# jeremy-rifkin/Markov-Huffman-Coding

Hardware: AMD Instinct MI355X
Metric: encode+decode GB/s on 16 GB byte stream, bit-exact round-trip (higher is better)
Workload: dtype u8

## Files before the change

### markov-huffman-coding_amd/csrc/mh_tree.hip

```cpp
#include <hip/hip_runtime.h>
#include <stdint.h>

#include "mh_kernels.h"
#include "mh_model.hpp"

namespace mhk {

using mh::DEC16_LEAF;
using mh::DEC16_NULL;
using mh::TREE_LEAF;
using mh::TREE_STRIDE;

constexpr uint16_t NONE = 0xFFFF;

template <bool K64>
struct RegHeap {
    uint32_t klo[10], khi[10], itm[10];
    uint32_t hn = 0;

    static __device__ __forceinline__ uint32_t uni(uint32_t v) { return uint32_t(__builtin_amdgcn_readfirstlane(int(v))); }
    static __device__ __forceinline__ uint32_t rl(uint32_t v, uint32_t lane) { return uint32_t(__builtin_amdgcn_readlane(int(v), int(lane))); }
    static __device__ __forceinline__ uint32_t wl(uint32_t val, uint32_t lane, uint32_t old) {
#pragma clang diagnostic push
#pragma clang diagnostic ignored "-Winline-asm"
        asm("s_mov_b32 m0, %2\n\tv_writelane_b32 %0, %1, m0" : "+v"(old) : "s"(uni(val)), "s"(uni(lane)) : "m0");
#pragma clang diagnostic pop
        return old;
    }
    static __device__ __forceinline__ bool lt(uint32_t alo, uint32_t ahi, uint32_t blo, uint32_t bhi) {
        if (K64) return ahi < bhi || (ahi == bhi && alo < blo);
        return alo < blo;
    }
    template <int L>
    __device__ __forceinline__ void get(uint32_t pos, uint32_t &lo, uint32_t &hi, uint32_t &it) const {
        if constexpr (L < 7) {
            lo = rl(klo[L], pos); hi = K64 ? rl(khi[L], pos) : 0u; it = rl(itm[L], pos);
        } else if constexpr (L == 7) {
            const uint32_t ln = pos & 63u;
            const bool up = pos >= 64u;
            lo = up ? rl(klo[8], ln) : rl(klo[7], ln);
            hi = K64 ? (up ? rl(khi[8], ln) : rl(khi[7], ln)) : 0u;
            it = up ? rl(itm[8], ln) : rl(itm[7], ln);
        } else {
            lo = rl(klo[9], 0); hi = K64 ? rl(khi[9], 0) : 0u; it = rl(itm[9], 0);
        }
    }
    template <int L>
    __device__ __forceinline__ void put(uint32_t pos, uint32_t lo, uint32_t hi, uint32_t it) {
        if constexpr (L < 7) {
            klo[L] = wl(lo, pos, klo[L]); if (K64) khi[L] = wl(hi, pos, khi[L]); itm[L] = wl(it, pos, itm[L]);
        } else if constexpr (L == 7) {
            const uint32_t ln = pos & 63u;
            if (pos >= 64u) { klo[8] = wl(lo, ln, klo[8]); if (K64) khi[8] = wl(hi, ln, khi[8]); itm[8] = wl(it, ln, itm[8]); }
            else { klo[7] = wl(lo, ln, klo[7]); if (K64) khi[7] = wl(hi, ln, khi[7]); itm[7] = wl(it, ln, itm[7]); }
        } else {
            klo[9] = wl(lo, 0, klo[9]); if (K64) khi[9] = wl(hi, 0, khi[9]); itm[9] = wl(it, 0, itm[9]);
        }
    }

    template <int L>
    __device__ __forceinline__ void swim_flat(uint32_t pos, uint32_t lo, uint32_t hi, uint32_t it) {
        uint32_t alo[L + 1], ahi[L + 1], ait[L + 1];
        uint32_t moves = 0;
        bool going = true;
        alo[L] = lo; ahi[L] = hi; ait[L] = it;
#pragma unroll
        for (int l = L - 1; l >= 0; --l) {
            get_dyn(l, pos >> (L - l), alo[l], ahi[l], ait[l]);
            going = going && lt(lo, hi, alo[l], ahi[l]);
            moves += going ? 1u : 0u;
        }
        const uint32_t f = uint32_t(L) - moves;
#pragma unroll
        for (int l = L; l >= 0; --l) {
            const bool from_parent = uint32_t(l) > f;
            const bool self = uint32_t(l) < f;
            const uint32_t plo = l > 0 ? alo[l > 0 ? l - 1 : 0] : lo, phi = l > 0 ? ahi[l > 0 ? l - 1 : 0] : hi,
                           pit = l > 0 ? ait[l > 0 ? l - 1 : 0] : it;
            const uint32_t wlo = from_parent ? plo : self ? alo[l] : lo;
            const uint32_t whi = from_parent ? phi : self ? ahi[l] : hi;
            const uint32_t wit = from_parent ? pit : self ? ait[l] : it;
            put_dyn(l, pos >> (L - l), wlo, whi, wit);
        }
    }
    template <int L>
    __device__ __forceinline__ void swim_short(uint32_t pos, uint32_t lo, uint32_t hi, uint32_t it) {
        uint32_t alo[L + 1], ahi[L + 1], ait[L + 1];
        uint32_t moves = 0;
#pragma unroll
        for (int l = L - 1; l >= 0; --l) {
            get_dyn(l, pos >> (L - l), alo[l], ahi[l], ait[l]);
            if (!lt(lo, hi, alo[l], ahi[l])) break;
            ++moves;
        }
#pragma unroll
        for (int m = 0; m < L; ++m) {
            if (uint32_t(m) < moves) put_dyn(L - m, pos >> m, alo[L - 1 - m], ahi[L - 1 - m], ait[L - 1 - m]);
        }
        put_any_level<L>(L - moves, pos >> moves, lo, hi, it);
    }
    template <int L>
    __device__ __forceinline__ void put_any_level(uint32_t level, uint32_t pos, uint32_t lo, uint32_t hi, uint32_t it) {
        switch (level) {
            case 0: put<0>(pos, lo, hi, it); break;
            case 1: if (L >= 1) put<1>(pos, lo, hi, it); break;
            case 2: if (L >= 2) put<2>(pos, lo, hi, it); break;
            case 3: if (L >= 3) put<3>(pos, lo, hi, it); break;
            case 4: if (L >= 4) put<4>(pos, lo, hi, it); break;
            case 5: if (L >= 5) put<5>(pos, lo, hi, it); break;
            case 6: if (L >= 6) put<6>(pos, lo, hi, it); break;
            case 7: if (L >= 7) put<7>(pos, lo, hi, it); break;
            default: if (L >= 8) put<8>(pos, lo, hi, it); break;
        }
    }
    __device__ __forceinline__ void get_dyn(int l, uint32_t pos, uint32_t &lo, uint32_t &hi, uint32_t &it) const {
        switch (l) {
            case 0: get<0>(pos, lo, hi, it); break; case 1: get<1>(pos, lo, hi, it); break; case 2: get<2>(pos, lo, hi, it); break;
            case 3: get<3>(pos, lo, hi, it); break; case 4: get<4>(pos, lo, hi, it); break; case 5: get<5>(pos, lo, hi, it); break;
            case 6: get<6>(pos, lo, hi, it); break; case 7: get<7>(pos, lo, hi, it); break; default: get<8>(pos, lo, hi, it); break;
        }
    }
    __device__ __forceinline__ void put_dyn(int l, uint32_t pos, uint32_t lo, uint32_t hi, uint32_t it) {
        switch (l) {
            case 0: put<0>(pos, lo, hi, it); break; case 1: put<1>(pos, lo, hi, it); break; case 2: put<2>(pos, lo, hi, it); break;
            case 3: put<3>(pos, lo, hi, it); break; case 4: put<4>(pos, lo, hi, it); break; case 5: put<5>(pos, lo, hi, it); break;
            case 6: put<6>(pos, lo, hi, it); break; case 7: put<7>(pos, lo, hi, it); break; default: put<8>(pos, lo, hi, it); break;
        }
    }
    __device__ __forceinline__ void push(uint32_t lo, uint32_t hi, uint32_t it) {
        const uint32_t i = hn++;
        const uint32_t level = 31u - uint32_t(__builtin_clz(i + 1u));
        const uint32_t pos = i + 1u - (1u << level);
        switch (level) {
            case 0: swim_short<0>(pos, lo, hi, it); break;
            case 1: swim_short<1>(pos, lo, hi, it); break;
            case 2: swim_short<2>(pos, lo, hi, it); break;
            case 3: swim_short<3>(pos, lo, hi, it); break;
            case 4: swim_short<4>(pos, lo, hi, it); break;
            case 5: swim_short<5>(pos, lo, hi, it); break;
            case 6: swim_short<6>(pos, lo, hi, it); break;
            case 7: swim_short<7>(pos, lo, hi, it); break;
            default: swim_short<8>(pos, lo, hi, it); break;
        }
    }
    template <int LMAX>
    __device__ __forceinline__ void sink_flat(uint32_t lo, uint32_t hi, uint32_t it) {
        uint32_t pos[LMAX + 1], clo[LMAX + 1], chi[LMAX + 1], cit[LMAX + 1];
        pos[0] = 0; clo[0] = lo; chi[0] = hi; cit[0] = it;
        uint32_t moves = 0;
        bool going = true;
#pragma unroll
        for (int l = 0; l < LMAX; ++l) {
            const uint32_t li = ((2u << l) - 1u) + 2u * pos[l];
            uint32_t llo, lhi, lit, rlo, rhi, rit;
            get_dyn(l + 1, 2u * pos[l], llo, lhi, lit);
            get_dyn(l + 1, 2u * pos[l] + 1u, rlo, rhi, rit);
            const bool right = li + 1u < hn && lt(rlo, rhi, llo, lhi);
            clo[l + 1] = right ? rlo : llo; chi[l + 1] = right ? rhi : lhi; cit[l + 1] = right ? rit : lit;
            pos[l + 1] = 2u * pos[l] + (right ? 1u : 0u);
            going = going && li < hn && lt(clo[l + 1], chi[l + 1], lo, hi);
            moves += going ? 1u : 0u;
        }
#pragma unroll
        for (int l = 0; l <= LMAX; ++l) {
            const bool from_child = uint32_t(l) < moves;
            const bool self = uint32_t(l) > moves;
            const int c = l < LMAX ? l + 1 : LMAX;
            const uint32_t wlo = from_child ? clo[c] : self ? clo[l] : lo;
            const uint32_t whi = from_child ? chi[c] : self ? chi[l] : hi;
            const uint32_t wit = from_child ? cit[c] : self ? cit[l] : it;
            put_dyn(l, pos[l], wlo, whi, wit);
        }
    }
    __device__ __forceinline__ uint32_t pop(uint32_t &mlo, uint32_t &mhi) {
        uint32_t top;
        get<0>(0, mlo, mhi, top);
        --hn;
        const uint32_t level = 31u - uint32_t(__builtin_clz(hn + 1u));
        const uint32_t pos = hn + 1u - (1u << level);
        uint32_t lo, hi, it;
        switch (level) {
            case 0: get<0>(pos, lo, hi, it); sink_flat<0>(lo, hi, it); break;
            case 1: get<1>(pos, lo, hi, it); sink_flat<1>(lo, hi, it); break;
            case 2: get<2>(pos, lo, hi, it); sink_flat<2>(lo, hi, it); break;
            case 3: get<3>(pos, lo, hi, it); sink_flat<3>(lo, hi, it); break;
            case 4: get<4>(pos, lo, hi, it); sink_flat<4>(lo, hi, it); break;
            case 5: get<5>(pos, lo, hi, it); sink_flat<5>(lo, hi, it); break;
            case 6: get<6>(pos, lo, hi, it); sink_flat<6>(lo, hi, it); break;
            case 7: get<7>(pos, lo, hi, it); sink_flat<7>(lo, hi, it); break;
            default: get<8>(pos, lo, hi, it); sink_flat<8>(lo, hi, it); break;
        }
        return top;
    }
};

struct TreeLds {
    uint16_t *left, *right, *parent, *height;
    uint8_t *sym;
    unsigned long long *weight;
};

template <bool K64>
__device__ __forceinline__ void merge_context(const TreeLds &t, uint32_t nleaf, uint32_t lane, uint32_t &nn_out, uint32_t &root_out,
                                              uint32_t &single_out) {
    RegHeap<K64> h;
#pragma unroll
    for (int i = 0; i < 10; ++i) { h.klo[i] = 0; h.khi[i] = 0; h.itm[i] = 0; }
    for (uint32_t i = 0; i < nleaf; ++i) {
        const unsigned long long w = t.weight[i];
        h.push(RegHeap<K64>::uni(uint32_t(w)), RegHeap<K64>::uni(uint32_t(w >> 32)), i);
    }
    uint32_t nn = nleaf;
    while (h.hn > 1) {
        uint32_t alo, ahi, blo, bhi;
        uint32_t a = h.pop(alo, ahi), b = h.pop(blo, bhi);
        if ((a >> 16) > (b >> 16)) {
            uint32_t x = a; a = b; b = x;
        }
        const unsigned long long w = ((unsigned long long)(ahi) << 32 | alo) + ((unsigned long long)(bhi) << 32 | blo);
        const uint32_t ha = a >> 16, hb = b >> 16, hnew = (ha > hb ? ha : hb) + 1u;
        const uint32_t ia = a & 0xFFFFu, ib = b & 0xFFFFu;
        if (lane == 0) {
            t.left[nn] = uint16_t(ia); t.right[nn] = uint16_t(ib); t.parent[nn] = NONE; t.sym[nn] = 0;
            t.weight[nn] = w; t.height[nn] = uint16_t(hnew);
            t.parent[ia] = t.parent[ib] = uint16_t(nn);
        }
        h.push(uint32_t(w), uint32_t(w >> 32), nn | (hnew << 16));
        ++nn;
    }
    uint32_t rlo, rhi;
    const uint32_t root = h.pop(rlo, rhi) & 0xFFFFu;
    single_out = 0;
    if (nleaf == 1) {
        if (lane == 0) {
            const uint8_t s = t.sym[root];
            for (int k = 0; k < 2; ++k) {
                t.left[nn + k] = t.right[nn + k] = NONE; t.parent[nn + k] = uint16_t(root); t.height[nn + k] = 0; t.sym[nn + k] = s;
                t.weight[nn + k] = t.weight[root];
            }
            t.left[root] = uint16_t(nn); t.right[root] = uint16_t(nn + 1);
            t.height[root] = 1;
        }
        nn += 2;
        single_out = 1;
    }
    nn_out = nn;
    root_out = root;
}

__global__ __launch_bounds__(64) void tree_build_kernel(const unsigned long long *__restrict__ counts, TreeBuildOut o) {
    const uint32_t c = blockIdx.x, lane = threadIdx.x;
    __shared__ unsigned long long cnt[256];
    __shared__ uint16_t left[TB_NODE_STRIDE], right[TB_NODE_STRIDE], parent[TB_NODE_STRIDE], height[TB_NODE_STRIDE];
    __shared__ uint8_t sym[TB_NODE_STRIDE];
    __shared__ unsigned long long weight[TB_NODE_STRIDE];
    __shared__ uint8_t olen[256];
    __shared__ unsigned long long ocode[256];
    __shared__ uint32_t prof[9];
    __shared__ uint32_t s_nn, s_root, s_single, s_ntab8, s_maxlen;

    unsigned long long wsum = 0;
    for (uint32_t i = lane; i < 256; i += 64) {
        cnt[i] = counts[size_t(c) * 256 + i];
        wsum += cnt[i];
        olen[i] = 0;
        ocode[i] = 0;
    }
    for (int d = 32; d >= 1; d >>= 1) wsum += __shfl_xor(wsum, d);
    if (lane < 9) prof[lane] = 0;
    if (lane == 0) { s_ntab8 = 0; s_maxlen = 0; s_single = 0; }
    __syncthreads();

    uint32_t nleaf = 0;
    for (uint32_t i = 0; i < 4; ++i) {
        const uint32_t s = i * 64 + lane;
        const bool nz = cnt[s] != 0;
        const unsigned long long m = __ballot(nz);
        const uint32_t pos = nleaf + __popcll(m & ((1ull << lane) - 1ull));
        if (nz) {
            left[pos] = right[pos] = NONE; parent[pos] = NONE; height[pos] = 0; sym[pos] = uint8_t(s); weight[pos] = cnt[s];
        }
        nleaf += __popcll(m);
    }
    __syncthreads();
    {
        const TreeLds t{left, right, parent, height, sym, weight};
        uint32_t nn = 0, root = 0xFFFFFFFFu, single = 0;
        if (nleaf > 0) {
            const bool wide = uint32_t(__builtin_amdgcn_readfirstlane(int(uint32_t(wsum >> 32)))) != 0;
            if (wide) merge_context<true>(t, nleaf, lane, nn, root, single);
            else merge_context<false>(t, nleaf, lane, nn, root, single);
        }
        if (lane == 0) { s_nn = nn; s_root = root; s_single = single; }
    }
    __syncthreads();

    const uint32_t nn = s_nn, root = s_root;
    if (root != 0xFFFFFFFFu) {
        for (uint32_t node = lane; node < nn; node += 64) {
            uint32_t d = 0;
            unsigned long long code = 0;
            uint32_t cur = node;
            while (cur != root) {
                const uint32_t p = parent[cur];
                if (right[p] == cur && d < 64) code |= 1ull << d;
                ++d;
                cur = p;
            }
            if (left[node] == NONE) {
                if (!(s_single && node == left[root])) {
                    olen[sym[node]] = uint8_t(d > 255 ? 255 : d);
                    ocode[sym[node]] = d <= 64 ? code : 0;
                    atomicMax(&s_maxlen, d);
                }
            } else if (d <= 8) {
                const uint32_t h = height[node] < o.hcap ? height[node] : o.hcap;
                atomicAdd(&prof[d], 1u << h);
                if (d == 8) atomicAdd(&s_ntab8, 1u);
            }
        }
    }
    __syncthreads();

    uint32_t lenmask = 0;
    for (uint32_t s = lane; s < 256; s += 64) {
        const uint32_t l = olen[s];
        if (l) lenmask |= 1u << (l < 32u ? l - 1u : 31u);
        const unsigned long long cd = ocode[s];
        o.len8[c * 256 + s] = uint8_t(l);
        o.code64[c * 256 + s] = cd;
        if (o.enc16) {
            const uint32_t slot = mh::enc_slot((s << 8) | c);
            uint16_t e = 0;
            if (l > uint32_t(mh::ENC16_MAX_LEN)) e = mh::ENC16_ESCAPE;
            else if (l > 0) e = uint16_t((l << 12) | uint32_t(cd));
            o.enc16[slot] = e;
            o.len_slot[slot] = uint8_t(l);
        }
    }
    for (uint32_t i = lane; i < TB_NODE_STRIDE; i += 64) {
        const bool live = i < nn;
        o.node_left[c * TB_NODE_STRIDE + i] = live ? left[i] : NONE;
        o.node_right[c * TB_NODE_STRIDE + i] = live ? right[i] : NONE;
        o.node_sym[c * TB_NODE_STRIDE + i] = live ? sym[i] : 0;
        o.node_height[c * TB_NODE_STRIDE + i] = live ? uint8_t(height[i] > 255 ? 255 : height[i]) : 0;
    }
    for (int d = 32; d >= 1; d >>= 1) lenmask |= __shfl_xor(lenmask, d);
    if (lane == 0) {
        uint32_t *m = o.ctx_meta + c * TB_META_STRIDE;
        m[0] = nn; m[1] = root; m[2] = s_maxlen; m[3] = s_ntab8;
        for (int d = 0; d < 9; ++d) m[4 + d] = prof[d];
        m[13] = uint32_t(wsum); m[14] = uint32_t(wsum >> 32);
        m[15] = nleaf < 2 ? 0u : lenmask;
    }
}

__device__ __forceinline__ void tree_pack_body(const TreePackArgs &a, const uint32_t c) {
    const uint32_t tid = threadIdx.x;
    __shared__ uint16_t left[TB_NODE_STRIDE], right[TB_NODE_STRIDE], nid[TB_NODE_STRIDE];
    __shared__ uint8_t sym[TB_NODE_STRIDE], height[TB_NODE_STRIDE];
    __shared__ uint32_t tr[TREE_STRIDE];
    __shared__ uint32_t scan[256];
    const uint32_t *meta = a.ctx_meta + c * TB_META_STRIDE;
    const uint32_t nn = meta[0], root = meta[1];
    for (uint32_t i = tid; i < TB_NODE_STRIDE; i += 256) {
        left[i] = a.node_left[c * TB_NODE_STRIDE + i];
        right[i] = a.node_right[c * TB_NODE_STRIDE + i];
        sym[i] = a.node_sym[c * TB_NODE_STRIDE + i];
        height[i] = a.node_height[c * TB_NODE_STRIDE + i];
    }
    tr[tid] = 0;
    __syncthreads();
    const uint32_t P = a.P, nprim = 1u << P;
    const uint32_t my_base = a.sec_base_in ? a.sec_base_in[c] : a.sec_base_val[c];
    if (tid == 0 && !a.sec_base_in && a.sec_base) a.sec_base[c] = my_base;
    if (root == 0xFFFFFFFFu) {
        if (tid < nprim) a.prim[(c << P) | tid] = DEC16_NULL;
        if (a.tree) a.tree[c * TREE_STRIDE + tid] = 0;
        return;
    }
    if (tid == 0) {
        uint32_t next = 1;
        for (uint32_t i = 0; i < nn; ++i) nid[i] = (left[i] == NONE) ? NONE : (i == root ? 0 : uint16_t(next++));
    }
    __syncthreads();
    auto enc_child = [&](uint32_t ch) -> uint32_t { return left[ch] == NONE ? (TREE_LEAF | sym[ch]) : uint32_t(nid[ch]); };
    for (uint32_t i = tid; i < nn; i += 256)
        if (left[i] != NONE) tr[nid[i]] = (enc_child(right[i]) << 16) | enc_child(left[i]);

    uint32_t node = root, depth = 0, tabsize = 0, h = 0;
    if (tid < nprim) {
        while (depth < P && left[node] != NONE) {
            const uint32_t bit = a.lsb ? (tid >> depth) & 1u : (tid >> (P - 1 - depth)) & 1u;
            node = bit ? right[node] : left[node];
            ++depth;
        }
        if (left[node] != NONE) {
            h = a.direct ? a.H : (height[node] < a.hcap ? height[node] : a.hcap);
            tabsize = 1u << h;
        }
    }
    scan[tid] = tabsize;
    __syncthreads();
    for (uint32_t d = 1; d < 256; d <<= 1) {
        uint32_t v = tid >= d ? scan[tid - d] : 0;
        __syncthreads();
        scan[tid] += v;
        __syncthreads();
    }
    const uint32_t off = scan[tid] - tabsize;
    const uint32_t base = my_base;
    if (tid < nprim) {
        uint16_t e;
        if (left[node] == NONE) e = uint16_t(DEC16_LEAF | (depth << 8) | sym[node]);
        else if (a.direct) e = uint16_t((base >> a.H) + (off >> a.H));
        else e = uint16_t(((h - 1) << 12) | off);
        a.prim[(c << P) | tid] = e;
        for (uint32_t x = 0; x < tabsize; ++x) {
            uint32_t n2 = node, d2 = 0;
            while (d2 < h && left[n2] != NONE) {
                const uint32_t bit = a.lsb ? (x >> d2) & 1u : (x >> (h - 1 - d2)) & 1u;
                n2 = bit ? right[n2] : left[n2];
                ++d2;
            }
            a.sec[base + off + x] = left[n2] == NONE ? uint16_t(DEC16_LEAF | ((P + d2) << 8) | sym[n2]) : uint16_t(nid[n2]);
        }
    }
    __syncthreads();
    if (a.tree) a.tree[c * TREE_STRIDE + tid] = tr[tid];
}

__global__ __launch_bounds__(256) void tree_pack_kernel(TreePackArgs a) { tree_pack_body(a, blockIdx.x); }
__global__ __launch_bounds__(256) void tree_pack2_kernel(TreePackArgs a, TreePackArgs b, uint32_t nctx) {
    if (blockIdx.x < nctx) tree_pack_body(a, blockIdx.x);
    else tree_pack_body(b, blockIdx.x - nctx);
}

__global__ __launch_bounds__(64) void o2_hot_pack_kernel(O2HotArgs a) {
    const uint32_t slot = blockIdx.x, lane = threadIdx.x;
    if (slot == a.nslots) { a.hot[slot * 64u + lane] = mh::ENC16_ESCAPE; return; }
    const uint32_t ctx = a.slot_ctx[slot];
    {
        uint16_t e = mh::ENC16_ESCAPE;
        if (lane < 63 && a.id_used[lane]) {
            const uint32_t k = ctx * 256u + a.id_sym[lane];
            const uint32_t l = a.len8[k];
            e = l == 0 ? uint16_t(0) : (l > uint32_t(mh::ENC16_MAX_LEN) ? mh::ENC16_ESCAPE : uint16_t((l << 12) | uint32_t(a.code64[k])));
        }
        a.hot[slot * 64u + (lane ^ a.slot_id1[slot])] = e;
    }
    if (!a.tprim) return;
    const uint32_t P = a.P, H = a.H;
    const uint16_t *left = a.node_left + size_t(ctx) * TB_NODE_STRIDE, *right = a.node_right + size_t(ctx) * TB_NODE_STRIDE;
    const uint8_t *sym = a.node_sym + size_t(ctx) * TB_NODE_STRIDE;
    const uint32_t root = a.ctx_meta[size_t(ctx) * TB_META_STRIDE + 1];
    auto leaf_entry = [&](uint32_t node, uint32_t len) -> uint32_t {
        const uint32_t s = sym[node];
        uint32_t nxt = a.ctx2slot[((ctx & 255u) << 8) | s];
        if (nxt == 0xFFFFu) nxt = 0;
        return (nxt << 16) | DEC16_LEAF | (len << 8) | s;
    };
    for (uint32_t w = lane; w < (1u << P); w += 64u) {
        uint32_t node = root, depth = 0;
        if (root != 0xFFFFFFFFu)
            while (depth < P && left[node] != NONE) { node = ((w >> depth) & 1u) ? right[node] : left[node]; ++depth; }
        const bool inner = root != 0xFFFFFFFFu && left[node] != NONE;
        const unsigned long long m = __ballot(inner);
        const uint32_t rank = uint32_t(__popcll(m & ((1ull << lane) - 1ull)));
        const uint32_t id = (slot << P) + rank;
        uint32_t e = DEC16_NULL;
        if (root != 0xFFFFFFFFu) e = inner ? id : leaf_entry(node, depth);
        a.tprim[(slot << P) + (w ^ (slot & ((1u << P) - 1u)))] = e;
        if (inner) {
            for (uint32_t x = 0; x < (1u << H); ++x) {
                uint32_t n2 = node, d2 = 0;
                while (d2 < H && left[n2] != NONE) { n2 = ((x >> d2) & 1u) ? right[n2] : left[n2]; ++d2; }
                a.tsec[(size_t(id) << H) + x] = left[n2] == NONE ? leaf_entry(n2, P + d2) : 0u;
            }
        }
    }
}

hipError_t launch_o2_hot_pack(const O2HotArgs &a, hipStream_t st) {
    hipLaunchKernelGGL(o2_hot_pack_kernel, dim3(a.nslots + 1), dim3(64), 0, st, a);
    return hipGetLastError();
}

hipError_t launch_tree_build(const unsigned long long *d_counts, int nctx, const TreeBuildOut &o, hipStream_t st) {
    hipLaunchKernelGGL(tree_build_kernel, dim3(nctx), dim3(64), 0, st, d_counts, o);
    return hipGetLastError();
}

hipError_t launch_tree_pack(const TreePackArgs &a, int nctx, hipStream_t st) {
    hipLaunchKernelGGL(tree_pack_kernel, dim3(nctx), dim3(256), 0, st, a);
    return hipGetLastError();
}
hipError_t launch_tree_pack2(const TreePackArgs &a, const TreePackArgs &b, int nctx, hipStream_t st) {
    hipLaunchKernelGGL(tree_pack2_kernel, dim3(2 * nctx), dim3(256), 0, st, a, b, uint32_t(nctx));
    return hipGetLastError();
}

}
```

Before: 535.9.

## Move Huffman tree-build heap from lane registers to LDS with wave-parallel sift

Replaces the register-resident heap (readlane/writelane per level, with switch dispatch on level) with a 1-indexed heap in shared memory. Push and pop use all 64 lanes to read the root-to-leaf path at once, find the insertion point with a ballot/popcount, and write the shifted entries in one parallel store. The aim is to cut the serial readlane/writelane chains and branchy dispatch in per-context tree construction. In exchange it adds LDS traffic and extra shared memory per block, and it only affects the tree-build phase, which is a small share of encode+decode time.

```diff
diff --git a/markov-huffman-coding_amd/csrc/mh_tree.hip b/markov-huffman-coding_amd/csrc/mh_tree.hip
--- a/markov-huffman-coding_amd/csrc/mh_tree.hip
+++ b/markov-huffman-coding_amd/csrc/mh_tree.hip
@@ -1,5 +1,7 @@
 #include <hip/hip_runtime.h>
 #include <stdint.h>
+
+#include <type_traits>
 
 #include "mh_kernels.h"
 #include "mh_model.hpp"
@@ -13,184 +15,57 @@
 
 constexpr uint16_t NONE = 0xFFFF;
 
+constexpr uint32_t HEAP_SPARE = 256, HEAP_SLOTS = 320;
+
 template <bool K64>
-struct RegHeap {
-    uint32_t klo[10], khi[10], itm[10];
+struct LdsHeap {
+    using Key = typename std::conditional<K64, unsigned long long, uint32_t>::type;
+    struct alignas(K64 ? 16 : 8) Ent {
+        Key key;
+        uint32_t item;
+    };
+    Ent *e;
+    uint32_t lane;
     uint32_t hn = 0;
 
     static __device__ __forceinline__ uint32_t uni(uint32_t v) { return uint32_t(__builtin_amdgcn_readfirstlane(int(v))); }
-    static __device__ __forceinline__ uint32_t rl(uint32_t v, uint32_t lane) { return uint32_t(__builtin_amdgcn_readlane(int(v), int(lane))); }
-    static __device__ __forceinline__ uint32_t wl(uint32_t val, uint32_t lane, uint32_t old) {
-#pragma clang diagnostic push
-#pragma clang diagnostic ignored "-Winline-asm"
-        asm("s_mov_b32 m0, %2\n\tv_writelane_b32 %0, %1, m0" : "+v"(old) : "s"(uni(val)), "s"(uni(lane)) : "m0");
-#pragma clang diagnostic pop
-        return old;
-    }
-    static __device__ __forceinline__ bool lt(uint32_t alo, uint32_t ahi, uint32_t blo, uint32_t bhi) {
-        if (K64) return ahi < bhi || (ahi == bhi && alo < blo);
-        return alo < blo;
-    }
-    template <int L>
-    __device__ __forceinline__ void get(uint32_t pos, uint32_t &lo, uint32_t &hi, uint32_t &it) const {
-        if constexpr (L < 7) {
-            lo = rl(klo[L], pos); hi = K64 ? rl(khi[L], pos) : 0u; it = rl(itm[L], pos);
-        } else if constexpr (L == 7) {
-            const uint32_t ln = pos & 63u;
-            const bool up = pos >= 64u;
-            lo = up ? rl(klo[8], ln) : rl(klo[7], ln);
-            hi = K64 ? (up ? rl(khi[8], ln) : rl(khi[7], ln)) : 0u;
-            it = up ? rl(itm[8], ln) : rl(itm[7], ln);
-        } else {
-            lo = rl(klo[9], 0); hi = K64 ? rl(khi[9], 0) : 0u; it = rl(itm[9], 0);
-        }
-    }
-    template <int L>
-    __device__ __forceinline__ void put(uint32_t pos, uint32_t lo, uint32_t hi, uint32_t it) {
-        if constexpr (L < 7) {
-            klo[L] = wl(lo, pos, klo[L]); if (K64) khi[L] = wl(hi, pos, khi[L]); itm[L] = wl(it, pos, itm[L]);
-        } else if constexpr (L == 7) {
-            const uint32_t ln = pos & 63u;
-            if (pos >= 64u) { klo[8] = wl(lo, ln, klo[8]); if (K64) khi[8] = wl(hi, ln, khi[8]); itm[8] = wl(it, ln, itm[8]); }
-            else { klo[7] = wl(lo, ln, klo[7]); if (K64) khi[7] = wl(hi, ln, khi[7]); itm[7] = wl(it, ln, itm[7]); }
-        } else {
-            klo[9] = wl(lo, 0, klo[9]); if (K64) khi[9] = wl(hi, 0, khi[9]); itm[9] = wl(it, 0, itm[9]);
-        }
-    }
-
-    template <int L>
-    __device__ __forceinline__ void swim_flat(uint32_t pos, uint32_t lo, uint32_t hi, uint32_t it) {
-        uint32_t alo[L + 1], ahi[L + 1], ait[L + 1];
-        uint32_t moves = 0;
-        bool going = true;
-        alo[L] = lo; ahi[L] = hi; ait[L] = it;
+    static __device__ __forceinline__ Key uni_key(Key k) {
+        if constexpr (K64) return (Key(uni(uint32_t(k >> 32))) << 32) | uni(uint32_t(k));
+        else return uni(k);
+    }
+
+    __device__ __forceinline__ void push(Key k, uint32_t it) {
+        const uint32_t n = ++hn;
+        const uint32_t L = 31u - uint32_t(__builtin_clz(n));
+        const uint32_t an = lane <= L ? n >> (L - lane) : HEAP_SPARE + lane;
+        const Ent a = e[an];
+        const Ent p = e[an >> 1];
+        const uint32_t f = L - uint32_t(__popcll(__ballot(lane < L && a.key > k)));
+        const bool self = lane == f, down = lane > f && lane <= L;
+        e[an] = Ent{self ? k : down ? p.key : a.key, self ? it : down ? p.item : a.item};
+    }
+
+    __device__ __forceinline__ uint32_t pop(Key &mkey) {
+        const Ent top = e[1];
+        const Ent last = e[hn];
+        --hn;
+        const Ent l0 = e[2u * lane], r0 = e[2u * lane + 1u], l1 = e[128u + 2u * lane], r1 = e[129u + 2u * lane];
+        const unsigned long long pa = __ballot(2u * lane + 1u <= hn && r0.key < l0.key);
+        const unsigned long long pb = __ballot(129u + 2u * lane <= hn && r1.key < l1.key);
+        mkey = uni_key(top.key);
+        const uint32_t titem = uni(top.item);
+        if (hn == 0) return titem;
+        uint32_t n = 1;
 #pragma unroll
-        for (int l = L - 1; l >= 0; --l) {
-            get_dyn(l, pos >> (L - l), alo[l], ahi[l], ait[l]);
-            going = going && lt(lo, hi, alo[l], ahi[l]);
-            moves += going ? 1u : 0u;
-        }
-        const uint32_t f = uint32_t(L) - moves;
-#pragma unroll
-        for (int l = L; l >= 0; --l) {
-            const bool from_parent = uint32_t(l) > f;
-            const bool self = uint32_t(l) < f;
-            const uint32_t plo = l > 0 ? alo[l > 0 ? l - 1 : 0] : lo, phi = l > 0 ? ahi[l > 0 ? l - 1 : 0] : hi,
-                           pit = l > 0 ? ait[l > 0 ? l - 1 : 0] : it;
-            const uint32_t wlo = from_parent ? plo : self ? alo[l] : lo;
-            const uint32_t whi = from_parent ? phi : self ? ahi[l] : hi;
-            const uint32_t wit = from_parent ? pit : self ? ait[l] : it;
-            put_dyn(l, pos >> (L - l), wlo, whi, wit);
-        }
-    }
-    template <int L>
-    __device__ __forceinline__ void swim_short(uint32_t pos, uint32_t lo, uint32_t hi, uint32_t it) {
-        uint32_t alo[L + 1], ahi[L + 1], ait[L + 1];
-        uint32_t moves = 0;
-#pragma unroll
-        for (int l = L - 1; l >= 0; --l) {
-            get_dyn(l, pos >> (L - l), alo[l], ahi[l], ait[l]);
-            if (!lt(lo, hi, alo[l], ahi[l])) break;
-            ++moves;
-        }
-#pragma unroll
-        for (int m = 0; m < L; ++m) {
-            if (uint32_t(m) < moves) put_dyn(L - m, pos >> m, alo[L - 1 - m], ahi[L - 1 - m], ait[L - 1 - m]);
-        }
-        put_any_level<L>(L - moves, pos >> moves, lo, hi, it);
-    }
-    template <int L>
-    __device__ __forceinline__ void put_any_level(uint32_t level, uint32_t pos, uint32_t lo, uint32_t hi, uint32_t it) {
-        switch (level) {
-            case 0: put<0>(pos, lo, hi, it); break;
-            case 1: if (L >= 1) put<1>(pos, lo, hi, it); break;
-            case 2: if (L >= 2) put<2>(pos, lo, hi, it); break;
-            case 3: if (L >= 3) put<3>(pos, lo, hi, it); break;
-            case 4: if (L >= 4) put<4>(pos, lo, hi, it); break;
-            case 5: if (L >= 5) put<5>(pos, lo, hi, it); break;
-            case 6: if (L >= 6) put<6>(pos, lo, hi, it); break;
-            case 7: if (L >= 7) put<7>(pos, lo, hi, it); break;
-            default: if (L >= 8) put<8>(pos, lo, hi, it); break;
-        }
-    }
-    __device__ __forceinline__ void get_dyn(int l, uint32_t pos, uint32_t &lo, uint32_t &hi, uint32_t &it) const {
-        switch (l) {
-            case 0: get<0>(pos, lo, hi, it); break; case 1: get<1>(pos, lo, hi, it); break; case 2: get<2>(pos, lo, hi, it); break;
-            case 3: get<3>(pos, lo, hi, it); break; case 4: get<4>(pos, lo, hi, it); break; case 5: get<5>(pos, lo, hi, it); break;
-            case 6: get<6>(pos, lo, hi, it); break; case 7: get<7>(pos, lo, hi, it); break; default: get<8>(pos, lo, hi, it); break;
-        }
-    }
-    __device__ __forceinline__ void put_dyn(int l, uint32_t pos, uint32_t lo, uint32_t hi, uint32_t it) {
-        switch (l) {
-            case 0: put<0>(pos, lo, hi, it); break; case 1: put<1>(pos, lo, hi, it); break; case 2: put<2>(pos, lo, hi, it); break;
-            case 3: put<3>(pos, lo, hi, it); break; case 4: put<4>(pos, lo, hi, it); break; case 5: put<5>(pos, lo, hi, it); break;
-            case 6: put<6>(pos, lo, hi, it); break; case 7: put<7>(pos, lo, hi, it); break; default: put<8>(pos, lo, hi, it); break;
-        }
-    }
-    __device__ __forceinline__ void push(uint32_t lo, uint32_t hi, uint32_t it) {
-        const uint32_t i = hn++;
-        const uint32_t level = 31u - uint32_t(__builtin_clz(i + 1u));
-        const uint32_t pos = i + 1u - (1u << level);
-        switch (level) {
-            case 0: swim_short<0>(pos, lo, hi, it); break;
-            case 1: swim_short<1>(pos, lo, hi, it); break;
-            case 2: swim_short<2>(pos, lo, hi, it); break;
-            case 3: swim_short<3>(pos, lo, hi, it); break;
-            case 4: swim_short<4>(pos, lo, hi, it); break;
-            case 5: swim_short<5>(pos, lo, hi, it); break;
-            case 6: swim_short<6>(pos, lo, hi, it); break;
-            case 7: swim_short<7>(pos, lo, hi, it); break;
-            default: swim_short<8>(pos, lo, hi, it); break;
-        }
-    }
-    template <int LMAX>
-    __device__ __forceinline__ void sink_flat(uint32_t lo, uint32_t hi, uint32_t it) {
-        uint32_t pos[LMAX + 1], clo[LMAX + 1], chi[LMAX + 1], cit[LMAX + 1];
-        pos[0] = 0; clo[0] = lo; chi[0] = hi; cit[0] = it;
-        uint32_t moves = 0;
-        bool going = true;
-#pragma unroll
-        for (int l = 0; l < LMAX; ++l) {
-            const uint32_t li = ((2u << l) - 1u) + 2u * pos[l];
-            uint32_t llo, lhi, lit, rlo, rhi, rit;
-            get_dyn(l + 1, 2u * pos[l], llo, lhi, lit);
-            get_dyn(l + 1, 2u * pos[l] + 1u, rlo, rhi, rit);
-            const bool right = li + 1u < hn && lt(rlo, rhi, llo, lhi);
-            clo[l + 1] = right ? rlo : llo; chi[l + 1] = right ? rhi : lhi; cit[l + 1] = right ? rit : lit;
-            pos[l + 1] = 2u * pos[l] + (right ? 1u : 0u);
-            going = going && li < hn && lt(clo[l + 1], chi[l + 1], lo, hi);
-            moves += going ? 1u : 0u;
-        }
-#pragma unroll
-        for (int l = 0; l <= LMAX; ++l) {
-            const bool from_child = uint32_t(l) < moves;
-            const bool self = uint32_t(l) > moves;
-            const int c = l < LMAX ? l + 1 : LMAX;
-            const uint32_t wlo = from_child ? clo[c] : self ? clo[l] : lo;
-            const uint32_t whi = from_child ? chi[c] : self ? chi[l] : hi;
-            const uint32_t wit = from_child ? cit[c] : self ? cit[l] : it;
-            put_dyn(l, pos[l], wlo, whi, wit);
-        }
-    }
-    __device__ __forceinline__ uint32_t pop(uint32_t &mlo, uint32_t &mhi) {
-        uint32_t top;
-        get<0>(0, mlo, mhi, top);
-        --hn;
-        const uint32_t level = 31u - uint32_t(__builtin_clz(hn + 1u));
-        const uint32_t pos = hn + 1u - (1u << level);
-        uint32_t lo, hi, it;
-        switch (level) {
-            case 0: get<0>(pos, lo, hi, it); sink_flat<0>(lo, hi, it); break;
-            case 1: get<1>(pos, lo, hi, it); sink_flat<1>(lo, hi, it); break;
-            case 2: get<2>(pos, lo, hi, it); sink_flat<2>(lo, hi, it); break;
-            case 3: get<3>(pos, lo, hi, it); sink_flat<3>(lo, hi, it); break;
-            case 4: get<4>(pos, lo, hi, it); sink_flat<4>(lo, hi, it); break;
-            case 5: get<5>(pos, lo, hi, it); sink_flat<5>(lo, hi, it); break;
-            case 6: get<6>(pos, lo, hi, it); sink_flat<6>(lo, hi, it); break;
-            case 7: get<7>(pos, lo, hi, it); sink_flat<7>(lo, hi, it); break;
-            default: get<8>(pos, lo, hi, it); sink_flat<8>(lo, hi, it); break;
-        }
-        return top;
+        for (int l = 0; l < 7; ++l) n = 2u * n + uint32_t(((l < 6 ? pa : pb) >> (n & 63u)) & 1u);
+        const uint32_t pn = lane < 8u ? n >> (7u - lane) : HEAP_SPARE + lane;
+        const uint32_t cn = lane < 7u ? n >> (6u - lane) : pn;
+        const Ent pe = e[pn];
+        const Ent ce = e[cn];
+        const uint32_t moves = uint32_t(__popcll(__ballot(lane >= 1u && pn <= hn && pe.key < last.key)));
+        const bool up = lane < moves, here = lane == moves;
+        e[pn] = Ent{up ? ce.key : here ? last.key : pe.key, up ? ce.item : here ? last.item : pe.item};
+        return titem;
     }
 };
 
@@ -198,26 +73,27 @@
     uint16_t *left, *right, *parent, *height;
     uint8_t *sym;
     unsigned long long *weight;
+    uint4 *heap;
 };
 
 template <bool K64>
 __device__ __forceinline__ void merge_context(const TreeLds &t, uint32_t nleaf, uint32_t lane, uint32_t &nn_out, uint32_t &root_out,
                                               uint32_t &single_out) {
-    RegHeap<K64> h;
-#pragma unroll
-    for (int i = 0; i < 10; ++i) { h.klo[i] = 0; h.khi[i] = 0; h.itm[i] = 0; }
+    using Heap = LdsHeap<K64>;
+    using Key = typename Heap::Key;
+    Heap h{reinterpret_cast<typename Heap::Ent *>(t.heap), lane};
     for (uint32_t i = 0; i < nleaf; ++i) {
         const unsigned long long w = t.weight[i];
-        h.push(RegHeap<K64>::uni(uint32_t(w)), RegHeap<K64>::uni(uint32_t(w >> 32)), i);
+        h.push(Key(w), i);
     }
     uint32_t nn = nleaf;
     while (h.hn > 1) {
-        uint32_t alo, ahi, blo, bhi;
-        uint32_t a = h.pop(alo, ahi), b = h.pop(blo, bhi);
+        Key ka, kb;
+        uint32_t a = h.pop(ka), b = h.pop(kb);
         if ((a >> 16) > (b >> 16)) {
             uint32_t x = a; a = b; b = x;
         }
-        const unsigned long long w = ((unsigned long long)(ahi) << 32 | alo) + ((unsigned long long)(bhi) << 32 | blo);
+        const unsigned long long w = (unsigned long long)(ka) + (unsigned long long)(kb);
         const uint32_t ha = a >> 16, hb = b >> 16, hnew = (ha > hb ? ha : hb) + 1u;
         const uint32_t ia = a & 0xFFFFu, ib = b & 0xFFFFu;
         if (lane == 0) {
@@ -225,11 +101,11 @@
             t.weight[nn] = w; t.height[nn] = uint16_t(hnew);
             t.parent[ia] = t.parent[ib] = uint16_t(nn);
         }
-        h.push(uint32_t(w), uint32_t(w >> 32), nn | (hnew << 16));
+        h.push(Key(w), nn | (hnew << 16));
         ++nn;
     }
-    uint32_t rlo, rhi;
-    const uint32_t root = h.pop(rlo, rhi) & 0xFFFFu;
+    Key kr;
+    const uint32_t root = h.pop(kr) & 0xFFFFu;
     single_out = 0;
     if (nleaf == 1) {
         if (lane == 0) {
@@ -254,6 +130,7 @@
     __shared__ uint16_t left[TB_NODE_STRIDE], right[TB_NODE_STRIDE], parent[TB_NODE_STRIDE], height[TB_NODE_STRIDE];
     __shared__ uint8_t sym[TB_NODE_STRIDE];
     __shared__ unsigned long long weight[TB_NODE_STRIDE];
+    __shared__ uint4 heap[HEAP_SLOTS];
     __shared__ uint8_t olen[256];
     __shared__ unsigned long long ocode[256];
     __shared__ uint32_t prof[9];
@@ -284,7 +161,7 @@
     }
     __syncthreads();
     {
-        const TreeLds t{left, right, parent, height, sym, weight};
+        const TreeLds t{left, right, parent, height, sym, weight, heap};
         uint32_t nn = 0, root = 0xFFFFFFFFu, single = 0;
         if (nleaf > 0) {
             const bool wide = uint32_t(__builtin_amdgcn_readfirstlane(int(uint32_t(wsum >> 32)))) != 0;
```

Result: faster. 548.5, median of 6 (+2.3%).
